# bogus2000/anytime-3D-reconstruction

Measured on AMD Instinct MI355X. Metric: 32^3 voxel reconstructions/sec at batch=256; IoU delta vs reference, higher is better.
Workload: dtype bf16

## Files before the change

### anytime-3d-reconstruction_amd/csrc/conv_direct.hip

```cpp
#include "direct_common.h"

namespace {

constexpr int CD_CIN = 64, CD_COUT = 128;
constexpr int CD_RB = CD_CIN * 2;
constexpr int CD_PIECES = 51;
constexpr int CD_TILE = CD_PIECES * 1024;
constexpr int CD_WST = CD_COUT * 128;
constexpr int CD_NST = 3;
constexpr int CD_RING = 2 * CD_TILE;
constexpr int CD_DUMMY = CD_RING + CD_NST * CD_WST;
constexpr int CD_LDS = CD_DUMMY + 1024;
constexpr int CD_SP = CD_COUT * 2 + 16;

__global__ __launch_bounds__(512, 1) void conv_direct_kernel(const __bf16 *__restrict__ x, const __bf16 *__restrict__ w,
                                                             const float *__restrict__ scale, const float *__restrict__ shift,
                                                             void *__restrict__ y, int dout_log2, unsigned x_bytes, unsigned w_bytes,
                                                             int act, int out_fp8) {
    extern __shared__ __attribute__((aligned(16))) char smem[];
    const int tid = threadIdx.x, lane = tid & 63;
    const int wave = __builtin_amdgcn_readfirstlane(tid >> 6);
    const int wm = wave >> 1, wn = wave & 1;
    const int lo = dout_log2, no = 1 << lo, li = lo + 1, n = 1 << li;

// ... 126 lines not shown
#pragma unroll
        for (int nt = 0; nt < 2; ++nt)
#pragma unroll
            for (int g = 0; g < 4; ++g) shv[nt][g] = *reinterpret_cast<const f32x4 *>(shift + wn * 64 + nt * 32 + 8 * g + 4 * fh);
    }
    auto fill = VV_DIRECT_FILL32(CD_SP, wn * 64);
    auto with_out = [&](auto act_c) {
        if (out_fp8) fill(act_c, std::true_type{});
        else fill(act_c, std::false_type{});
    };
    VV_WITH_ACT(act, with_out);
    __syncthreads();
    vv_direct_store_box<512, CD_SP, CD_COUT, CD_COUT>(stage, y, box, lo, tid, out_fp8);
}

__global__ __launch_bounds__(512, 1) void conv_direct16_kernel(const __bf16 *__restrict__ x, const __bf16 *__restrict__ w,
                                                             const float *__restrict__ scale, const float *__restrict__ shift,
                                                             void *__restrict__ y, int dout_log2, unsigned x_bytes, unsigned w_bytes,
                                                             int act, int out_fp8) {
    extern __shared__ __attribute__((aligned(16))) char smem[];
    const int tid = threadIdx.x, lane = tid & 63;
    const int wave = __builtin_amdgcn_readfirstlane(tid >> 6);
    const int wm = wave >> 1, wn = wave & 1;
    const int lo = dout_log2, no = 1 << lo, li = lo + 1, n = 1 << li;

    const VvDirectBox box = vv_direct_box(no);
    const int b = box.b, od0 = box.od0, oh0 = box.oh0, ow0 = box.ow0;

    const u32x4 rsx = vv_make_rsrc(x, x_bytes), rsw = vv_make_rsrc(w, w_bytes);
    const unsigned lds0 = (unsigned)(unsigned long long)(lptr_t)smem;
// ... 20 lines not shown
            const int g = (lane & 7) ^ ((row >> 1) & 7);
            const unsigned vo = c < 64 ? (unsigned)row * (64 * CD_RB) + t * CD_RB + g * 16 : 0xFFFFFFF0u;
            vv_dma16(rsw, vo, st + (wave * 2 + i) * 1024);
        }
    };

#pragma unroll 1
    for (int s = 0; s < 7; ++s) issue_x(0, s);
    issue_w(0);
    issue_w(1);
    issue_w(2);
    vv_wait_vm<0>();
    __syncthreads();

    const int r = lane & 15, kq = lane >> 4;
    const int rl0 = wm * 81 + (r >> 3) * 9 + (r & 7);
    unsigned xo[2][2], wo[2];
#pragma unroll
    for (int aw = 0; aw < 2; ++aw)
#pragma unroll
        for (int ks = 0; ks < 2; ++ks) xo[aw][ks] = lds0 + rl0 * CD_RB + (((ks * 4 + kq) ^ ((2 * ((r & 7) + aw)) & 7)) << 4);
#pragma unroll
    for (int ks = 0; ks < 2; ++ks) wo[ks] = lds0 + CD_RING + (wn * 64 + r) * 128 + (((ks * 4 + kq) ^ ((r >> 1) & 7)) << 4);

    f32x4 acc[4][4];
#pragma unroll
    for (int i = 0; i < 4; ++i)
#pragma unroll
        for (int j = 0; j < 4; ++j) acc[i][j] = f32x4{0.f, 0.f, 0.f, 0.f};

#define CD16_LD(F, XA, XOFF, WA)                                                                                                    \
// ... 3 lines not shown
                 : "=&v"(F[0]), "=&v"(F[1]), "=&v"(F[2]), "=&v"(F[3]), "=&v"(F[4]), "=&v"(F[5]), "=&v"(F[6]), "=&v"(F[7])            \
                 : "v"(XA), "v"(WA), "n"(XOFF), "n"((XOFF) + 2304), "n"((XOFF) + 4608), "n"((XOFF) + 6912)                          \
                 : "memory")
#define CD16_WAIT(F, N)                                                                                                             \
    asm volatile("s_waitcnt lgkmcnt(%8)"                                                                                            \
                 : "+v"(F[0]), "+v"(F[1]), "+v"(F[2]), "+v"(F[3]), "+v"(F[4]), "+v"(F[5]), "+v"(F[6]), "+v"(F[7])                    \
                 : "n"(N)                                                                                                           \
                 : "memory")
#define CD16_SB __builtin_amdgcn_sched_barrier(0)
#define CD16_RD(D, A, OFF) asm volatile("ds_read_b128 %0, %1 offset:%2" : "=&v"(D) : "v"(A), "n"(OFF) : "memory")
#define CD16_MF(F, COT, CT)                                                                                                         \
    acc[COT][CT] = __builtin_amdgcn_mfma_f32_16x16x32_bf16(*reinterpret_cast<const bf16x8 *>(&F[4 + COT]),                          \
                                                           *reinterpret_cast<const bf16x8 *>(&F[CT]), acc[COT][CT], 0, 0, 0)

    u32x4 P[8], Q[8];
    CD16_LD(P, xo[0][0], 0, wo[0]);

#pragma unroll 1
    for (int q = 0; q < 8; ++q) {
        const unsigned tsel = (q & 1) * CD_TILE, tnext = ((q + 1) & 1) * CD_TILE;
        auto tap = [&](auto a_c) {
            constexpr int A = decltype(a_c)::value;
            constexpr int AW = A & 1, TO = (((A >> 2) & 1) * 81 + ((A >> 1) & 1) * 9 + AW) * CD_RB;
            constexpr int AN = (A + 1) & 7, AWN = AN & 1, TON = (((AN >> 2) & 1) * 81 + ((AN >> 1) & 1) * 9 + AWN) * CD_RB;
            const int c = q * 8 + A;
            const unsigned wsel = (c % CD_NST) * CD_WST, wnext = ((c + 1) % CD_NST) * CD_WST;
            const unsigned xq = xo[AW][1] + tsel, wq = wo[1] + wsel;
            CD16_WAIT(P, 0);
            CD16_SB;
            CD16_MF(P, 0, 0); CD16_MF(P, 0, 1); CD16_SB; CD16_RD(Q[0], xq, TO); CD16_RD(Q[4], wq, 0); CD16_SB;
            CD16_MF(P, 0, 2); CD16_MF(P, 0, 3); CD16_SB; CD16_RD(Q[1], xq, TO + 2304); CD16_RD(Q[5], wq, 2048); CD16_SB;
            CD16_MF(P, 1, 0); CD16_MF(P, 1, 1); CD16_SB; CD16_RD(Q[2], xq, TO + 4608); CD16_RD(Q[6], wq, 4096); CD16_SB;
            CD16_MF(P, 1, 2); CD16_MF(P, 1, 3); CD16_SB; CD16_RD(Q[3], xq, TO + 6912); CD16_RD(Q[7], wq, 6144); CD16_SB;
            CD16_MF(P, 2, 0); CD16_MF(P, 2, 1); CD16_MF(P, 2, 2); CD16_MF(P, 2, 3);
            CD16_MF(P, 3, 0); CD16_MF(P, 3, 1); CD16_MF(P, 3, 2); CD16_MF(P, 3, 3);
            CD16_SB;
            CD16_WAIT(Q, 0);
            vv_wait_vm<(A == 0 || A == 7) ? 2 : 3>();
            __syncthreads();
            CD16_SB;
            CD16_MF(Q, 0, 0); CD16_MF(Q, 0, 1);
// ... 22 lines not shown
    vv_wait_vm<0>();
    __syncthreads();

    char *stage = smem;
    f32x4 scv[4], shv[4];
#pragma unroll
    for (int cot = 0; cot < 4; ++cot) { scv[cot] = f32x4{1.f, 1.f, 1.f, 1.f}; shv[cot] = f32x4{0.f, 0.f, 0.f, 0.f}; }
    if (scale) {
#pragma unroll
        for (int cot = 0; cot < 4; ++cot) scv[cot] = *reinterpret_cast<const f32x4 *>(scale + wn * 64 + cot * 16 + 4 * kq);
    }
    if (shift) {
#pragma unroll
        for (int cot = 0; cot < 4; ++cot) shv[cot] = *reinterpret_cast<const f32x4 *>(shift + wn * 64 + cot * 16 + 4 * kq);
    }
    auto fill = VV_DIRECT_FILL16(CD_SP, wn * 64);
    auto with_out = [&](auto act_c) {
        if (out_fp8) fill(act_c, std::true_type{});
        else fill(act_c, std::false_type{});
    };
    VV_WITH_ACT(act, with_out);
    __syncthreads();
    vv_direct_store_box<512, CD_SP, CD_COUT, CD_COUT>(stage, y, box, lo, tid, out_fp8);
}


constexpr int CDH_COUT = 64;
constexpr int CDH_WST = CDH_COUT * 128;
constexpr int CDH_RING = CD_TILE;
constexpr int CDH_DUMMY = CDH_RING + CD_NST * CDH_WST;
constexpr int CDH_LDS = CDH_DUMMY + 1024;
// ... 136 lines not shown
    vv_wait_vm<0>();
    __syncthreads();

    char *stage = smem;
    f32x4 scv[4], shv[4];
#pragma unroll
    for (int cot = 0; cot < 4; ++cot) { scv[cot] = f32x4{1.f, 1.f, 1.f, 1.f}; shv[cot] = f32x4{0.f, 0.f, 0.f, 0.f}; }
    if (scale) {
#pragma unroll
        for (int cot = 0; cot < 4; ++cot) scv[cot] = *reinterpret_cast<const f32x4 *>(scale + nh * CDH_COUT + cot * 16 + 4 * kq);
    }
    if (shift) {
#pragma unroll
        for (int cot = 0; cot < 4; ++cot) shv[cot] = *reinterpret_cast<const f32x4 *>(shift + nh * CDH_COUT + cot * 16 + 4 * kq);
    }
    auto fill = VV_DIRECT_FILL16(CDH_SP, 0);
    auto with_out = [&](auto act_c) {
        if (out_fp8) fill(act_c, std::true_type{});
        else fill(act_c, std::false_type{});
    };
    VV_WITH_ACT(act, with_out);
    __syncthreads();
    vv_direct_store_box<256, CDH_SP, CDH_COUT, CD_COUT>(stage, y, box, lo, tid, out_fp8);
}


}

VV_EXPORT int vv_conv3d_k4s2_direct_supported(int side, int cin, int cout, int dtype) {
    return dtype == VV_BF16 && cin == CD_CIN && cout == CD_COUT && side >= 16 && vv_is_pow2(side);
}

VV_EXPORT int vv_conv3d_k4s2_direct_fwd_io(const void *x, const void *w_packed, const float *scale, const float *shift, void *y,
                                           int batch, int side, int cin, int cout, int act, int dtype, int out_dtype, void *stream) {
    if (!x || !w_packed || !y) return VV_ERR_NULL;
    if (out_dtype != VV_BF16 && out_dtype != VV_FP8) return VV_ERR_DTYPE;
    if (!vv_conv3d_k4s2_direct_supported(side, cin, cout, dtype) || batch <= 0) return VV_ERR_SHAPE;
    if (!vv_aligned16(x) || !vv_aligned16(w_packed) || !vv_aligned16(y)) return VV_ERR_ALIGN;
    const int so = side / 2;
    const int boxes = (so / 4) * (so / 8) * (so / 8);
    vv_allow_lds<&conv_direct_kernel>(CD_LDS);
    vv_allow_lds<&conv_direct16_kernel>(CD_LDS);
    vv_allow_lds<&conv_direct16h_kernel>(CDH_LDS);
    const int shape = vv_hook_int(vv_hook("VV_CD_SHAPE"), 16);
    const bool s16 = shape != 32, half = shape == 8;
    const size_t in_per = (size_t)side * side * side * cin * 2, out_per = (size_t)so * so * so * cout * (out_dtype == VV_FP8 ? 1 : 2);
    const int per = vv_chunk_samples(in_per, batch);
    if (per < 1) return VV_ERR_SHAPE;
    for (int b0 = 0; b0 < batch; b0 += per) {
        const int nb = batch - b0 < per ? batch - b0 : per;
        const __bf16 *xc = reinterpret_cast<const __bf16 *>(reinterpret_cast<const char *>(x) + (size_t)b0 * in_per);
        void *yc = reinterpret_cast<char *>(y) + (size_t)b0 * out_per;
        if (half)
            VV_LAUNCH(conv_direct16h_kernel, dim3(nb * boxes * 2), dim3(256), CDH_LDS, reinterpret_cast<hipStream_t>(stream), xc,
                      reinterpret_cast<const __bf16 *>(w_packed), scale, shift, yc, vv_log2(so), (unsigned)((size_t)nb * in_per),
                      (unsigned)((size_t)64 * cin * cout * 2), act, out_dtype == VV_FP8 ? 1 : 0,
                      vv_hook_int(vv_hook("VV_CDH_STAGGER"), 5), vv_hook_int(vv_hook("VV_CDH_ABL"), 0));
        else if (s16)
            VV_LAUNCH(conv_direct16_kernel, dim3(nb * boxes), dim3(512), CD_LDS, reinterpret_cast<hipStream_t>(stream), xc,
                      reinterpret_cast<const __bf16 *>(w_packed), scale, shift, yc, vv_log2(so), (unsigned)((size_t)nb * in_per),
                      (unsigned)((size_t)64 * cin * cout * 2), act, out_dtype == VV_FP8 ? 1 : 0);
        else
            VV_LAUNCH(conv_direct_kernel, dim3(nb * boxes), dim3(512), CD_LDS, reinterpret_cast<hipStream_t>(stream), xc,
                      reinterpret_cast<const __bf16 *>(w_packed), scale, shift, yc, vv_log2(so), (unsigned)((size_t)nb * in_per),
                      (unsigned)((size_t)64 * cin * cout * 2), act, out_dtype == VV_FP8 ? 1 : 0);
        const int rc = vv_launch_status();
        if (rc != VV_OK) return rc;
    }
    return VV_OK;
}

VV_EXPORT int vv_conv3d_k4s2_direct_fwd(const void *x, const void *w_packed, const float *scale, const float *shift, void *y,
                                        int batch, int side, int cin, int cout, int act, int dtype, void *stream) {
    return vv_conv3d_k4s2_direct_fwd_io(x, w_packed, scale, shift, y, batch, side, cin, cout, act, dtype, dtype, stream);
// ... 2 lines not shown
```

### anytime-3d-reconstruction_amd/csrc/convt_whole.hip

```cpp

#include <utility>

#include "common.h"

namespace {

constexpr int CW_X = 512 * 256;
constexpr int CW_WST = 64 * 128;
constexpr int CW_NST = 3;
constexpr int CW_RING = CW_X;
constexpr int CW_ZERO = CW_RING + CW_NST * CW_WST;
constexpr int CW_SS = CW_ZERO + 256;
constexpr int CW_LDS = CW_SS + 512;

#define CW_LD(F, X0, X1, WA)                                                                                                     \
    asm volatile("ds_read_b128 %0, %4\n\tds_read_b128 %1, %5\n\tds_read_b128 %2, %6\n\tds_read_b128 %3, %6 offset:4096"          \
                 : "=&v"(F[0]), "=&v"(F[1]), "=&v"(F[2]), "=&v"(F[3])                                                            \
                 : "v"(X0), "v"(X1), "v"(WA)                                                                                     \
                 : "memory")
#define CW_WAIT(F, N) asm volatile("s_waitcnt lgkmcnt(%4)" : "+v"(F[0]), "+v"(F[1]), "+v"(F[2]), "+v"(F[3]) : "n"(N) : "memory")
#define CW_MFMA4(F)                                                                                                              \
    do {                                                                                                                         \
        _Pragma("unroll") for (int nt = 0; nt < 2; ++nt) _Pragma("unroll") for (int mt = 0; mt < 2; ++mt)                        \
            acc[nt][mt] = __builtin_amdgcn_mfma_f32_32x32x16_bf16(*reinterpret_cast<const bf16x8 *>(&F[2 + nt]),                 \
// ... 182 lines not shown
                 "ds_read_b128 %7, %12 offset:6144"                                                                                 \
                 : "=&v"(F[0]), "=&v"(F[1]), "=&v"(F[2]), "=&v"(F[3]), "=&v"(F[4]), "=&v"(F[5]), "=&v"(F[6]), "=&v"(F[7])            \
                 : "v"(XA[0]), "v"(XA[1]), "v"(XA[2]), "v"(XA[3]), "v"(WA)                                                           \
                 : "memory")
#define CW16_WAIT(F, N)                                                                                                             \
    asm volatile("s_waitcnt lgkmcnt(%8)"                                                                                            \
                 : "+v"(F[0]), "+v"(F[1]), "+v"(F[2]), "+v"(F[3]), "+v"(F[4]), "+v"(F[5]), "+v"(F[6]), "+v"(F[7])                    \
                 : "n"(N)                                                                                                           \
                 : "memory")
#define CW16_SB __builtin_amdgcn_sched_barrier(0)
#define CW16_RD(D, A, OFF) asm volatile("ds_read_b128 %0, %1 offset:%2" : "=&v"(D) : "v"(A), "n"(OFF) : "memory")
#define CW16_MF(F, COT, CT)                                                                                                         \
    acc[COT][CT] = __builtin_amdgcn_mfma_f32_16x16x32_bf16(*reinterpret_cast<const bf16x8 *>(&F[4 + COT]),                          \
                                                           *reinterpret_cast<const bf16x8 *>(&F[CT]), acc[COT][CT], 0, 0, 0)

template <int ACT, bool STATS = false>
__global__ __launch_bounds__(512, 1) void ctw16_kernel(const __bf16 *__restrict__ x, const __bf16 *__restrict__ w,
                                                       const float *__restrict__ scale, const float *__restrict__ shift,
                                                       __bf16 *__restrict__ y, int npar, float *__restrict__ partial = nullptr) {
    extern __shared__ __attribute__((aligned(256))) char smem[];
    const int tid = threadIdx.x, lane = tid & 63;
    const int wave = __builtin_amdgcn_readfirstlane(tid >> 6);
    const int ps = 8 / npar;
    const int b = (int)blockIdx.x / ps, p0 = ((int)blockIdx.x % ps) * npar;
    const int NC = npar * 16;
    const unsigned lds0 = (unsigned)(unsigned long long)(lptr_t)smem;

    const u32x4 rsx = vv_make_rsrc(x + (size_t)b * (512 * 128), CW_X);
    const u32x4 rsw = vv_make_rsrc(w, 64 * 128 * 64 * 2);
    {
        const int pos = lane & 15, vsub = lane >> 4;
// ... 13 lines not shown
    issue_w(0, 0);
    issue_w(1, 1);
    issue_w(2, 2);
    if (tid < 16) *reinterpret_cast<uint4 *>(smem + CW_ZERO + tid * 16) = uint4{0u, 0u, 0u, 0u};
    if (tid >= 64 && tid < 128) {
        const int ch = tid - 64;
        *reinterpret_cast<float *>(smem + CW_SS + ch * 4) = scale ? scale[ch] : 1.f;
        *reinterpret_cast<float *>(smem + CW_SS + 256 + ch * 4) = shift ? shift[ch] : 0.f;
    }
    vv_wait_vm<0>();
    __syncthreads();

    const int r = lane & 15, q = lane >> 4;
    const int rh = r >> 3, rw = r & 7;
    const unsigned wl = lds0 + CW_RING + r * 128 + ((q ^ ((r >> 1) & 7)) << 4);
    const unsigned R0 = lds0 + (unsigned)((wave * 64 + r) << 8);
    const unsigned ZR = lds0 + CW_ZERO;
    auto tap_setup = [&](auto a_c, int pd, int ph, int pw, unsigned (&t)[4]) {
        constexpr int A = decltype(a_c)::value;
        const int dd = pd - ((A >> 2) & 1), dh = ph - ((A >> 1) & 1), dw = pw - (A & 1);
        const bool okw = (unsigned)(wave + dd) < 8u && (unsigned)(rw + dw) < 8u;
        const int sft = dd * 64 + dh * 8 + dw;
        const unsigned key = ((unsigned)((2 * (rw + dw)) ^ q) & 15u) << 4;
#pragma unroll
        for (int ct = 0; ct < 4; ++ct) {
            const unsigned row = okw && (unsigned)(2 * ct + rh + dh) < 8u ? R0 + (unsigned)((sft + 16 * ct) << 8) : ZR;
            t[ct] = row ^ key;
        }
    };

    f32x4 acc[4][4];
#pragma unroll
    for (int i = 0; i < 4; ++i)
#pragma unroll
        for (int j = 0; j < 4; ++j) acc[i][j] = f32x4{0.f, 0.f, 0.f, 0.f};
    f32x4 st1[4], st2[4];
#pragma unroll
    for (int i = 0; i < 4; ++i) { st1[i] = f32x4{0.f, 0.f, 0.f, 0.f}; st2[i] = f32x4{0.f, 0.f, 0.f, 0.f}; }

    auto epilogue = [&](int p) {
        const int pd = (p >> 2) & 1, ph = (p >> 1) & 1, pw = p & 1;
        const int qo = (q & 1) * 32 + (q >> 1) * 16;
        char *yb = reinterpret_cast<char *>(y) + ((((size_t)b * 16 + 2 * wave + pd) * 16 + 2 * rh + ph) * 16 + 2 * rw + pw) * 128 + qo;
        const char *ss = smem + CW_SS + q * 16;
#pragma unroll
        for (int c2 = 0; c2 < 2; ++c2) {
            u32x2 o[2][4];
#pragma unroll
            for (int h = 0; h < 2; ++h) {
                const int cot = 2 * c2 + h;
                const f32x4 sc = *reinterpret_cast<const f32x4 *>(ss + cot * 64);
                const f32x4 sh = *reinterpret_cast<const f32x4 *>(ss + 256 + cot * 64);
#pragma unroll
                for (int ct = 0; ct < 4; ++ct) {
                    const f32x4 t = vv_bn_act4<ACT>(acc[cot][ct], sc, sh);
                    bf16x4 v;
#pragma unroll
                    for (int e = 0; e < 4; ++e) v[e] = static_cast<__bf16>(t[e]);
                    if (STATS) {
                        const f32x4 f = {(float)v[0], (float)v[1], (float)v[2], (float)v[3]};
                        st1[cot] += f;
                        st2[cot] += f * f;
                    }
                    acc[cot][ct] = f32x4{0.f, 0.f, 0.f, 0.f};
                    o[h][ct] = *reinterpret_cast<const u32x2 *>(&v);
                }
            }
#pragma unroll
            for (int ct = 0; ct < 4; ++ct) {
                auto rx = __builtin_amdgcn_permlane16_swap(o[0][ct][0], o[1][ct][0], false, false);
                auto ry = __builtin_amdgcn_permlane16_swap(o[0][ct][1], o[1][ct][1], false, false);
                *reinterpret_cast<u32x4 *>(yb + (size_t)(ct * 4 * 16 * 128) + c2 * 64) = u32x4{rx[0], ry[0], rx[1], ry[1]};
            }
        }
    };

    u32x4 P[8], Q[8];
    unsigned ua[4], ub[4];
    tap_setup(std::integral_constant<int, 0>{}, (p0 >> 2) & 1, (p0 >> 1) & 1, p0 & 1, ua);
    unsigned ws = wl;
    int stg = 0, cw = 3;
    CW16_LD(P, ua, ws);
#pragma unroll 1
    for (int pi = 0; pi < npar; ++pi) {
        const int p = p0 + pi, pd = (p >> 2) & 1, ph = (p >> 1) & 1, pw = p & 1;
        const int pn = p + 1, pnd = (pn >> 2) & 1, pnh = (pn >> 1) & 1, pnw = pn & 1;
        auto chunk = [&](auto j_c) {
            constexpr int J = decltype(j_c)::value, A = J >> 1, KH = J & 1;
            unsigned xq[4];
#pragma unroll
            for (int ct = 0; ct < 4; ++ct) xq[ct] = ua[ct] ^ (KH ? 192u : 64u);
            const unsigned wq = ws ^ 64u;
            CW16_WAIT(P, 0);
            CW16_SB;
            CW16_MF(P, 0, 0); CW16_MF(P, 0, 1); CW16_SB; CW16_RD(Q[0], xq[0], 0); CW16_RD(Q[4], wq, 0); CW16_SB;
            CW16_MF(P, 0, 2); CW16_MF(P, 0, 3); CW16_SB; CW16_RD(Q[1], xq[1], 0); CW16_RD(Q[5], wq, 2048); CW16_SB;
            CW16_MF(P, 1, 0); CW16_MF(P, 1, 1); CW16_SB; CW16_RD(Q[2], xq[2], 0); CW16_RD(Q[6], wq, 4096); CW16_SB;
            CW16_MF(P, 1, 2); CW16_MF(P, 1, 3); CW16_SB; CW16_RD(Q[3], xq[3], 0); CW16_RD(Q[7], wq, 6144); CW16_SB;
            CW16_MF(P, 2, 0); CW16_MF(P, 2, 1); CW16_MF(P, 2, 2); CW16_MF(P, 2, 3);
            if (KH == 0) {
                if (A < 7) tap_setup(std::integral_constant<int, (A + 1) & 7>{}, pd, ph, pw, ub);
                else tap_setup(std::integral_constant<int, 0>{}, pnd, pnh, pnw, ub);
// ... 13 lines not shown
            if (KH == 0) {
#pragma unroll
                for (int ct = 0; ct < 4; ++ct) xq[ct] = ua[ct] ^ 128u;
            } else {
#pragma unroll
                for (int ct = 0; ct < 4; ++ct) xq[ct] = ua[ct] = ub[ct];
            }
            CW16_SB;
            CW16_MF(Q, 0, 2); CW16_MF(Q, 0, 3); CW16_SB; CW16_RD(P[0], xq[0], 0); CW16_RD(P[4], ws, 0); CW16_SB;
            CW16_MF(Q, 1, 0); CW16_MF(Q, 1, 1); CW16_SB; CW16_RD(P[1], xq[1], 0); CW16_RD(P[5], ws, 2048); CW16_SB;
            CW16_MF(Q, 1, 2); CW16_MF(Q, 1, 3); CW16_SB; CW16_RD(P[2], xq[2], 0); CW16_RD(P[6], ws, 4096); CW16_SB;
            CW16_MF(Q, 2, 0); CW16_MF(Q, 2, 1); CW16_SB; CW16_RD(P[3], xq[3], 0); CW16_RD(P[7], ws, 6144); CW16_SB;
            CW16_MF(Q, 2, 2); CW16_MF(Q, 2, 3);
            CW16_MF(Q, 3, 0); CW16_MF(Q, 3, 1); CW16_MF(Q, 3, 2); CW16_MF(Q, 3, 3);
            CW16_SB;
        };
        chunk(std::integral_constant<int, 0>{});
        chunk(std::integral_constant<int, 1>{});
        chunk(std::integral_constant<int, 2>{});
        chunk(std::integral_constant<int, 3>{});
        chunk(std::integral_constant<int, 4>{});
        chunk(std::integral_constant<int, 5>{});
        chunk(std::integral_constant<int, 6>{});
        chunk(std::integral_constant<int, 7>{});
        chunk(std::integral_constant<int, 8>{});
        chunk(std::integral_constant<int, 9>{});
        chunk(std::integral_constant<int, 10>{});
        chunk(std::integral_constant<int, 11>{});
        chunk(std::integral_constant<int, 12>{});
        chunk(std::integral_constant<int, 13>{});
// ... 332 lines not shown
    if (!vv_convT3d_k4s2_whole_supported(side, cin, cout, dtype) || batch <= 0) return VV_ERR_SHAPE;
    if (!vv_aligned16(x) || !vv_aligned16(w_skip) || !vv_aligned16(y)) return VV_ERR_ALIGN;
    int ps = 1;
    while (ps < 8 && (long)batch * ps < 256) ps *= 2;
    if (const char *e = vv_hook("VV_CTW_PS")) {
        const int v = atoi(e);
        if (v == 1 || v == 2 || v == 4 || v == 8) ps = v;
    }
    const int shape = vv_hook_int(vv_hook("VV_CTW_SHAPE"), 16);
    const bool shape16 = shape != 32;
    hipStream_t st = reinterpret_cast<hipStream_t>(stream);
    auto launch = [&](auto act_c) {
        constexpr int ACT = decltype(act_c)::value;
        vv_allow_lds<&ctw_kernel<ACT>>(CW_LDS);
        vv_allow_lds<&ctw16_kernel<ACT>>(CW_LDS);
        vv_allow_lds<&ctw4_kernel<ACT>>(CW_LDS);
        if (shape != 16 && shape != 32)
            VV_LAUNCH(ctw4_kernel<ACT>, dim3((unsigned)batch * ps), dim3(256), CW_LDS, st, reinterpret_cast<const __bf16 *>(x),
                      reinterpret_cast<const __bf16 *>(w_skip), scale, shift, reinterpret_cast<__bf16 *>(y), 8 / ps);
        else if (shape16)
            VV_LAUNCH(ctw16_kernel<ACT>, dim3((unsigned)batch * ps), dim3(512), CW_LDS, st, reinterpret_cast<const __bf16 *>(x),
                      reinterpret_cast<const __bf16 *>(w_skip), scale, shift, reinterpret_cast<__bf16 *>(y), 8 / ps);
        else
            VV_LAUNCH(ctw_kernel<ACT>, dim3((unsigned)batch * ps), dim3(512), CW_LDS, st, reinterpret_cast<const __bf16 *>(x),
                      reinterpret_cast<const __bf16 *>(w_skip), scale, shift, reinterpret_cast<__bf16 *>(y), 8 / ps);
    };
    vv_with_act(act, launch);
    return vv_launch_status();
}

VV_EXPORT int vv_convT3d_k4s2_whole_stats_blocks(int batch) { return batch > 0 ? batch : 0; }

VV_EXPORT int vv_convT3d_k4s2_whole_stats_fwd(const void *x, const void *w_skip, void *y, float *stats_partial, size_t stats_bytes, int batch,
// ... 12 lines not shown
```

### anytime-3d-reconstruction_amd/csrc/direct_common.h

```cpp
#pragma once
#include "common.h"

struct VvDirectBox { int b, od0, oh0, ow0, nh; };

template <bool HALVES = false>
__device__ __forceinline__ VvDirectBox vv_direct_box(int no) {
    const int nwg = gridDim.x;
    int blk = (nwg & 7) == 0 ? (int)(blockIdx.x & 7) * (nwg >> 3) + (int)(blockIdx.x >> 3) : (int)blockIdx.x;
    VvDirectBox o;
    o.nh = 0;
    if (HALVES) { o.nh = blk & 1; blk >>= 1; }
    const int bxw = no >> 3, bxh = no >> 3, bxd = no >> 2;
    const int bw = blk % bxw; blk /= bxw;
    const int bh = blk % bxh; blk /= bxh;
    const int bd = blk % bxd;
    o.b = blk / bxd;
    o.od0 = bd * 4; o.oh0 = bh * 8; o.ow0 = bw * 8;
    return o;
}

#define VV_DIRECT_PUT4(dst, c, v)                                                                          \
    do {                                                                                                   \
        if (FP8) {                                                                                         \
            *reinterpret_cast<unsigned *>(dst + c) = vv_pack_fp8x4(v);                                     \
        } else {                                                                                           \
            bf16x4 o;                                                                                      \
            _Pragma("unroll") for (int e = 0; e < 4; ++e) o[e] = static_cast<__bf16>(v[e]);                \
            *reinterpret_cast<bf16x4 *>(dst + c * 2) = o;                                                  \
        }                                                                                                  \
    } while (0)

#define VV_DIRECT_FILL16(PITCH, C0)                                                                        \
    [&](auto act_c, auto fp8_c) {                                                                          \
        constexpr int ACT = decltype(act_c)::value;                                                        \
        constexpr bool FP8 = decltype(fp8_c)::value;                                                       \
        _Pragma("unroll") for (int ct = 0; ct < 4; ++ct)                                                   \
            _Pragma("unroll") for (int cot = 0; cot < 4; ++cot) {                                          \
                const int c = (C0) + cot * 16 + 4 * kq;                                                    \
                const f32x4 sc = scv[cot], sh = shv[cot];                                                  \
                const f32x4 v = vv_bn_act4<ACT>(acc[cot][ct], sc, sh);                                     \
                char *dst = stage + (wm * 64 + ct * 16 + r) * (PITCH);                                     \
                VV_DIRECT_PUT4(dst, c, v);                                                                 \
            }                                                                                              \
    }
#define VV_DIRECT_FILL32(PITCH, C0)                                                                        \
    [&](auto act_c, auto fp8_c) {                                                                          \
        constexpr int ACT = decltype(act_c)::value;                                                        \
        constexpr bool FP8 = decltype(fp8_c)::value;                                                       \
        _Pragma("unroll") for (int mt = 0; mt < 2; ++mt)                                                   \
            _Pragma("unroll") for (int nt = 0; nt < 2; ++nt)                                               \
                _Pragma("unroll") for (int g = 0; g < 4; ++g) {                                            \
                    const int c = (C0) + nt * 32 + 8 * g + 4 * fh;                                         \
                    const f32x4 sc = scv[nt][g], sh = shv[nt][g];                                          \
                    f32x4 v;                                                                               \
                    _Pragma("unroll") for (int e = 0; e < 4; ++e) {                                        \
                        float t = acc[nt][mt][4 * g + e] * sc[e] + sh[e];                                  \
// ... 23 lines not shown
```

### anytime-3d-reconstruction_amd/csrc/skip_direct.hip

```cpp
#include "common.h"

namespace {

typedef __attribute__((ext_vector_type(4))) unsigned sd_u4;

constexpr int SD_ATILE = 256 * 128;
constexpr int SD_WST = 32768;
constexpr int SD_A0 = 4096;
constexpr int SD_W0 = SD_A0 + 2 * SD_ATILE;
constexpr int SD_ZERO = SD_W0 + 2 * SD_WST;
constexpr int SD_LDS = SD_ZERO + 4096;
constexpr int SD_XCH = 0;
constexpr int SD_OST = 65536;
constexpr int SD_OPITCH = 144;
constexpr int SD_TPITCH = 272;
constexpr int SD_TWAVE = 16 * SD_TPITCH;

struct SdArgs {
    const void *x;
    const void *w;
    const float *scale;
    const float *shift;
    void *y;
    int batch, cin, cout, act;
// ... 86 lines not shown
}

__global__ void sd_pack_convT_multi_kernel(const SdPackJobs t) {
    int j = 0;
    while (j + 1 < t.njobs && (int)blockIdx.x >= t.first[j + 1]) ++j;
    sd_pack_convT_body(t.w[j], t.out[j], t.cin[j], t.cout[j], (int)blockIdx.x - t.first[j], t.first[j + 1] - t.first[j]);
}

#define SD_RD(DST, ADDR, OFF) asm volatile("ds_read_b128 %0, %1 offset:%2" : "=v"(DST) : "v"(ADDR), "n"(OFF) : "memory")
#define SD_WAIT8(N, F, G)                                                                                                   \
    asm volatile("s_waitcnt lgkmcnt(%8)"                                                                                    \
                 : "+v"(F[0]), "+v"(F[1]), "+v"(F[2]), "+v"(F[3]), "+v"(G[0]), "+v"(G[1]), "+v"(G[2]), "+v"(G[3])          \
                 : "n"(N)                                                                                                   \
                 : "memory")

template <int MODE>
__global__ __launch_bounds__(512, 1) void sd_kernel(const SdArgs a) {
    extern __shared__ __attribute__((aligned(16))) char smem[];
    const int tid = threadIdx.x, lane = tid & 63;
    const int wave = __builtin_amdgcn_readfirstlane(tid >> 6);
    const int mq = wave & 3, hv = wave >> 2;
    const int NC = a.cin >> 6;

    const int nwg = gridDim.x;
    const int wi = (nwg & 7) ? (int)blockIdx.x : (int)(blockIdx.x & 7) * (nwg >> 3) + (int)(blockIdx.x >> 3);
    const int sg = wi / a.groups, g = wi - sg * a.groups;
    const int b0 = sg * 4;
    const int ng = MODE == 0 ? g : (g >> 2);
    const int pd = (g >> 1) & 1, ph = g & 1;

    const u32x4 rsx = vv_make_rsrc(a.x, a.x_bytes), rsw = vv_make_rsrc(a.w, a.w_bytes);
    const unsigned lds0 = (unsigned)(unsigned long long)(lptr_t)smem;

    for (int i = tid; i < 256; i += 512) reinterpret_cast<uint4 *>(smem + SD_ZERO)[i] = make_uint4(0, 0, 0, 0);
    __syncthreads();

// ... 274 lines not shown
    __builtin_amdgcn_s_barrier();

    const int kq4 = kq * 4;
    if constexpr (MODE == 0) {
        f32x4 *xch = reinterpret_cast<f32x4 *>(smem + SD_XCH);
        {
            f32x4 *mine = xch + (size_t)wave * 8 * 64 + lane;
#pragma unroll
            for (int i = 0; i < 4; ++i)
#pragma unroll
                for (int j = 0; j < 2; ++j) mine[(i * 2 + j) * 64] = hv ? acc[i][j] : acc[i][2 + j];
        }
        __syncthreads();
        f32x4 fin[4][2];
        {
            const f32x4 *theirs = xch + (size_t)(wave ^ 4) * 8 * 64 + lane;
#pragma unroll
            for (int i = 0; i < 4; ++i)
#pragma unroll
                for (int j = 0; j < 2; ++j) fin[i][j] = (hv ? acc[i][2 + j] : acc[i][j]) + theirs[(i * 2 + j) * 64];
        }
        f32x4 sc[2], sh[2];
#pragma unroll
        for (int j = 0; j < 2; ++j) {
            const int n = ng * 64 + (2 * hv + j) * 16 + kq4;
            sc[j] = a.scale ? *reinterpret_cast<const f32x4 *>(a.scale + n) : f32x4{1.f, 1.f, 1.f, 1.f};
            sh[j] = a.shift ? *reinterpret_cast<const f32x4 *>(a.shift + n) : f32x4{0.f, 0.f, 0.f, 0.f};
        }
        auto fill = [&](auto act_c) {
            constexpr int ACT = decltype(act_c)::value;
#pragma unroll
// ... 60 lines not shown
                    if (b < a.batch)
                        *reinterpret_cast<uint4 *>(reinterpret_cast<char *>(a.y) + ((((size_t)b * 8 + od) * 8 + oh) * 8 + ow) * (a.cout * 2) + ng * 256 + pc * 16) =
                            *reinterpret_cast<const uint4 *>(mystage + row * SD_TPITCH + pc * 16);
                }
                asm volatile("s_waitcnt lgkmcnt(0)" ::: "memory");
                __builtin_amdgcn_wave_barrier();
            }
        };
        VV_WITH_ACT(a.act, fill);
    }
}

template <int MODE>
int sd_launch(const void *x, const void *w, const float *scale, const float *shift, void *y, int batch, int cin, int cout, int act,
              hipStream_t st) {
    vv_allow_lds<&sd_kernel<MODE>>(SD_LDS);
    const size_t in_vox = MODE == 0 ? 512 : 64, out_vox = MODE == 0 ? 64 : 512;
    const size_t sample_in = in_vox * cin * 2, sample_out = out_vox * cout * 2;
    int per = (int)((0x7FFFFFFFull / sample_in) & ~3ull);
    if (per < 4) return VV_ERR_SHAPE;
    for (int s0 = 0; s0 < batch; s0 += per) {
        const int nb = batch - s0 < per ? batch - s0 : per;
        SdArgs a;
        a.x = reinterpret_cast<const char *>(x) + (size_t)s0 * sample_in;
        a.y = reinterpret_cast<char *>(y) + (size_t)s0 * sample_out;
        a.w = w; a.scale = scale; a.shift = shift;
        a.batch = nb; a.cin = cin; a.cout = cout; a.act = act;
        a.x_bytes = (unsigned)((size_t)nb * sample_in);
        a.w_bytes = (unsigned)((size_t)64 * cin * cout * 2);
        a.groups = MODE == 0 ? cout / 64 : 4 * (cout / 128);
        const int nsg = (nb + 3) / 4;
        VV_LAUNCH(sd_kernel<MODE>, dim3(nsg * a.groups), dim3(512), SD_LDS, st, a);
        const int rc = vv_launch_status();
        if (rc != VV_OK) return rc;
    }
    return VV_OK;
}

}

VV_EXPORT int vv_conv3d_k4s2_skip_supported(int side, int cin, int cout, int dtype) {
    return dtype == VV_BF16 && side == 8 && cin >= 64 && cin % 64 == 0 && cout >= 64 && cout % 64 == 0 && (size_t)64 * cin * cout * 2 < 0xFFFFFFF0ull;
}

VV_EXPORT int vv_convT3d_k4s2_skip_supported(int side, int cin, int cout, int dtype) {
    return dtype == VV_BF16 && side == 4 && cin >= 64 && cin % 64 == 0 && cout >= 128 && cout % 128 == 0 && (size_t)64 * cin * cout * 2 < 0xFFFFFFF0ull;
}
// ... 78 lines not shown
```

### anytime-3d-reconstruction_amd/voxvae/lib.py

```python
import ctypes
import os

import torch

PKG = os.path.dirname(os.path.dirname(os.path.abspath(__file__)))
LIB_PATH = os.path.join(PKG, 'lib', 'libvoxvae.so')
HOOKS_LIB_PATH = os.path.join(PKG, 'lib', 'libvoxvae_hooks.so')
HOOK_VARS = ('VV_CD_SHAPE', 'VV_CDH_STAGGER', 'VV_CDH_ABL', 'VV_DIRECT_MT', 'VV_LT_KSLICE', 'VV_SPLIT_TARGET', 'VV_SPLIT_MINCHUNKS', 'VV_NO_KHALVES', 'VV_POSMAJOR_CONV_SIDE',
             'VV_POSMAJOR_CONVT_SIDE', 'VV_STAGES', 'VV_NO_FIRSTCONV', 'VV_WGRAD_F32', 'VV_PG_TARGET', 'VV_CTW_PS', 'VV_CTW_SHAPE',
             'VV_NO_WGRAD_PHASE', 'VV_BN_NB', 'VV_BN_SWEEP', 'VV_FINAL_BCE', 'VV_FIRSTCONV_GATHER', 'VV_FIRSTCONV_WGS', 'VV_FIRSTCONV_NOCHAIN', 'VV_CHUNK_SAMPLES')

VV_F32, VV_BF16, VV_FP8 = 0, 1, 2
ACT = {None: 0, 'None': 0, 'linear': 0, 'elu': 1, 'relu': 2, 'lrelu': 3}
DTYPES = {'f32': VV_F32, 'fp32': VV_F32, 'float32': VV_F32, 'bf16': VV_BF16, 'bfloat16': VV_BF16, 'fp8': VV_FP8}

_vp, _i, _f, _sz, _l = ctypes.c_void_p, ctypes.c_int, ctypes.c_float, ctypes.c_size_t, ctypes.c_long

SIGNATURES = {
    'vv_abi_version': (_i, []),
    'vv_status_string': (ctypes.c_char_p, [_i]),
    'vv_last_hip_error': (ctypes.c_char_p, []),
    'vv_pack_conv_k4': (_i, [_vp, _vp, _i, _i, _i, _vp]),
    'vv_pack_convT_k4s2': (_i, [_vp, _vp, _i, _i, _i, _vp]),
    'vv_pack_conv_k4s1_meanpool': (_i, [_vp, _vp, _i, _i, _i, _i, _vp]),
    'vv_pack_conv_k4s1_full': (_i, [_vp, _vp, _i, _i, _i, _i, _vp]),
# ... 151 lines not shown
```

Before: 560,700.

## Deal output tiles diagonally across waves to skip out-of-range boundary taps

The default 16-wide direct conv kernel now maps each wave's four column tiles onto rotated depth planes, so boundary planes are spread across waves. Whole MFMA groups for depth taps that fall outside the volume can then be skipped per wave instead of being multiplied against padding. The epilogue row mapping and LDS read addresses are rewritten to match. An opt-in diagonal variant of the transposed-conv kernel (shape hook 1) and a hook-gated wave remap for the skip kernel are also added; these add code paths and risk new LDS bank conflicts or branch overhead.

```diff
diff --git a/anytime-3d-reconstruction_amd/csrc/conv_direct.hip b/anytime-3d-reconstruction_amd/csrc/conv_direct.hip
--- a/anytime-3d-reconstruction_amd/csrc/conv_direct.hip
+++ b/anytime-3d-reconstruction_amd/csrc/conv_direct.hip
@@ -164,6 +164,7 @@
     vv_direct_store_box<512, CD_SP, CD_COUT, CD_COUT>(stage, y, box, lo, tid, out_fp8);
 }
 
+template <bool DEAL>
 __global__ __launch_bounds__(512, 1) void conv_direct16_kernel(const __bf16 *__restrict__ x, const __bf16 *__restrict__ w,
                                                              const float *__restrict__ scale, const float *__restrict__ shift,
                                                              void *__restrict__ y, int dout_log2, unsigned x_bytes, unsigned w_bytes,
@@ -214,7 +215,11 @@
     __syncthreads();
 
     const int r = lane & 15, kq = lane >> 4;
-    const int rl0 = wm * 81 + (r >> 3) * 9 + (r & 7);
+    const int rl0 = (DEAL ? 0 : wm * 81) + (r >> 3) * 9 + (r & 7);
+    int shp[4];
+    unsigned shb[4];
+#pragma unroll
+    for (int ct = 0; ct < 4; ++ct) { shp[ct] = DEAL ? (ct + wm) & 3 : ct; shb[ct] = (unsigned)(shp[ct] * 2304); }
     unsigned xo[2][2], wo[2];
 #pragma unroll
     for (int aw = 0; aw < 2; ++aw)
@@ -248,7 +253,14 @@
                                                            *reinterpret_cast<const bf16x8 *>(&F[CT]), acc[COT][CT], 0, 0, 0)
 
     u32x4 P[8], Q[8];
-    CD16_LD(P, xo[0][0], 0, wo[0]);
+    const bool skip_lo = DEAL && od0 == 0, skip_hi = DEAL && od0 + 4 == no;
+    if constexpr (DEAL) {
+        CD16_RD(P[0], xo[0][0] + shb[0], 0); CD16_RD(P[1], xo[0][0] + shb[1], 81 * CD_RB); CD16_RD(P[2], xo[0][0] + shb[2], 2 * 81 * CD_RB);
+        CD16_RD(P[3], xo[0][0] + shb[3], 3 * 81 * CD_RB);
+        CD16_RD(P[4], wo[0], 0); CD16_RD(P[5], wo[0], 2048); CD16_RD(P[6], wo[0], 4096); CD16_RD(P[7], wo[0], 6144);
+    } else {
+        CD16_LD(P, xo[0][0], 0, wo[0]);
+    }
 
 #pragma unroll 1
     for (int q = 0; q < 8; ++q) {
@@ -259,6 +271,41 @@
             constexpr int AN = (A + 1) & 7, AWN = AN & 1, TON = (((AN >> 2) & 1) * 81 + ((AN >> 1) & 1) * 9 + AWN) * CD_RB;
             const int c = q * 8 + A;
             const unsigned wsel = (c % CD_NST) * CD_WST, wnext = ((c + 1) % CD_NST) * CD_WST;
+            if constexpr (DEAL) {
+                constexpr int AD = (A >> 2) & 1, CS = AD ? 3 : 0, N0 = CS == 0 ? 1 : 0, N1 = N0 + 1, N2 = N0 + 2;
+                constexpr int PL = 81 * CD_RB;
+                const bool sk = AD ? skip_hi && (q & 4) : skip_lo && !(q & 4);
+                const unsigned xb = xo[AW][1] + tsel, wq = wo[1] + wsel;
+                const unsigned xq0 = xb + shb[0], xq1 = xb + shb[1], xq2 = xb + shb[2], xq3 = xb + shb[3];
+                CD16_WAIT(P, 0);
+                CD16_SB;
+                CD16_MF(P, 0, N0); CD16_MF(P, 0, N1); CD16_SB; CD16_RD(Q[0], xq0, TO); CD16_RD(Q[4], wq, 0); CD16_SB;
+                CD16_MF(P, 0, N2); CD16_MF(P, 1, N0); CD16_SB; CD16_RD(Q[1], xq1, TO + PL); CD16_RD(Q[5], wq, 2048); CD16_SB;
+                CD16_MF(P, 1, N1); CD16_MF(P, 1, N2); CD16_SB; CD16_RD(Q[2], xq2, TO + 2 * PL); CD16_RD(Q[6], wq, 4096); CD16_SB;
+                CD16_MF(P, 2, N0); CD16_MF(P, 2, N1); CD16_SB; CD16_RD(Q[3], xq3, TO + 3 * PL); CD16_RD(Q[7], wq, 6144); CD16_SB;
+                CD16_MF(P, 2, N2); CD16_MF(P, 3, N0); CD16_MF(P, 3, N1); CD16_MF(P, 3, N2);
+                CD16_SB;
+                if (!sk) { CD16_MF(P, 0, CS); CD16_MF(P, 1, CS); CD16_MF(P, 2, CS); CD16_MF(P, 3, CS); CD16_SB; }
+                CD16_WAIT(Q, 0);
+                vv_wait_vm<(A == 0 || A == 7) ? 2 : 3>();
+                __syncthreads();
+                CD16_SB;
+                CD16_MF(Q, 0, N0); CD16_MF(Q, 0, N1);
+                if (A < 7) issue_x(q + 1, A);
+                CD16_MF(Q, 0, N2); CD16_MF(Q, 1, N0);
+                issue_w(c + 3);
+                const unsigned xn = xo[AWN][0] + (A == 7 ? tnext : tsel), wp = wo[0] + wnext;
+                const unsigned xp0 = xn + shb[0], xp1 = xn + shb[1], xp2 = xn + shb[2], xp3 = xn + shb[3];
+                CD16_SB;
+                CD16_RD(P[0], xp0, TON); CD16_RD(P[4], wp, 0); CD16_SB;
+                CD16_MF(Q, 1, N1); CD16_MF(Q, 1, N2); CD16_SB; CD16_RD(P[1], xp1, TON + PL); CD16_RD(P[5], wp, 2048); CD16_SB;
+                CD16_MF(Q, 2, N0); CD16_MF(Q, 2, N1); CD16_SB; CD16_RD(P[2], xp2, TON + 2 * PL); CD16_RD(P[6], wp, 4096); CD16_SB;
+                CD16_MF(Q, 2, N2); CD16_MF(Q, 3, N0); CD16_SB; CD16_RD(P[3], xp3, TON + 3 * PL); CD16_RD(P[7], wp, 6144); CD16_SB;
+                CD16_MF(Q, 3, N1); CD16_MF(Q, 3, N2);
+                CD16_SB;
+                if (!sk) { CD16_MF(Q, 0, CS); CD16_MF(Q, 1, CS); CD16_MF(Q, 2, CS); CD16_MF(Q, 3, CS); CD16_SB; }
+                return;
+            }
             const unsigned xq = xo[AW][1] + tsel, wq = wo[1] + wsel;
             CD16_WAIT(P, 0);
             CD16_SB;
@@ -311,7 +358,7 @@
 #pragma unroll
         for (int cot = 0; cot < 4; ++cot) shv[cot] = *reinterpret_cast<const f32x4 *>(shift + wn * 64 + cot * 16 + 4 * kq);
     }
-    auto fill = VV_DIRECT_FILL16(CD_SP, wn * 64);
+    auto fill = VV_DIRECT_FILL16(CD_SP, wn * 64, (DEAL ? ct * 64 + shp[ct] * 16 : wm * 64 + ct * 16) + r);
     auto with_out = [&](auto act_c) {
         if (out_fp8) fill(act_c, std::true_type{});
         else fill(act_c, std::false_type{});
@@ -478,7 +525,7 @@
 #pragma unroll
         for (int cot = 0; cot < 4; ++cot) shv[cot] = *reinterpret_cast<const f32x4 *>(shift + nh * CDH_COUT + cot * 16 + 4 * kq);
     }
-    auto fill = VV_DIRECT_FILL16(CDH_SP, 0);
+    auto fill = VV_DIRECT_FILL16(CDH_SP, 0, wm * 64 + ct * 16 + r);
     auto with_out = [&](auto act_c) {
         if (out_fp8) fill(act_c, std::true_type{});
         else fill(act_c, std::false_type{});
@@ -504,7 +551,8 @@
     const int so = side / 2;
     const int boxes = (so / 4) * (so / 8) * (so / 8);
     vv_allow_lds<&conv_direct_kernel>(CD_LDS);
-    vv_allow_lds<&conv_direct16_kernel>(CD_LDS);
+    vv_allow_lds<&conv_direct16_kernel<true>>(CD_LDS);
+    vv_allow_lds<&conv_direct16_kernel<false>>(CD_LDS);
     vv_allow_lds<&conv_direct16h_kernel>(CDH_LDS);
     const int shape = vv_hook_int(vv_hook("VV_CD_SHAPE"), 16);
     const bool s16 = shape != 32, half = shape == 8;
@@ -520,8 +568,12 @@
                       reinterpret_cast<const __bf16 *>(w_packed), scale, shift, yc, vv_log2(so), (unsigned)((size_t)nb * in_per),
                       (unsigned)((size_t)64 * cin * cout * 2), act, out_dtype == VV_FP8 ? 1 : 0,
                       vv_hook_int(vv_hook("VV_CDH_STAGGER"), 5), vv_hook_int(vv_hook("VV_CDH_ABL"), 0));
+        else if (shape == 1)
+            VV_LAUNCH(conv_direct16_kernel<false>, dim3(nb * boxes), dim3(512), CD_LDS, reinterpret_cast<hipStream_t>(stream), xc,
+                      reinterpret_cast<const __bf16 *>(w_packed), scale, shift, yc, vv_log2(so), (unsigned)((size_t)nb * in_per),
+                      (unsigned)((size_t)64 * cin * cout * 2), act, out_dtype == VV_FP8 ? 1 : 0);
         else if (s16)
-            VV_LAUNCH(conv_direct16_kernel, dim3(nb * boxes), dim3(512), CD_LDS, reinterpret_cast<hipStream_t>(stream), xc,
+            VV_LAUNCH(conv_direct16_kernel<true>, dim3(nb * boxes), dim3(512), CD_LDS, reinterpret_cast<hipStream_t>(stream), xc,
                       reinterpret_cast<const __bf16 *>(w_packed), scale, shift, yc, vv_log2(so), (unsigned)((size_t)nb * in_per),
                       (unsigned)((size_t)64 * cin * cout * 2), act, out_dtype == VV_FP8 ? 1 : 0);
         else
diff --git a/anytime-3d-reconstruction_amd/csrc/convt_whole.hip b/anytime-3d-reconstruction_amd/csrc/convt_whole.hip
--- a/anytime-3d-reconstruction_amd/csrc/convt_whole.hip
+++ b/anytime-3d-reconstruction_amd/csrc/convt_whole.hip
@@ -220,7 +220,7 @@
     acc[COT][CT] = __builtin_amdgcn_mfma_f32_16x16x32_bf16(*reinterpret_cast<const bf16x8 *>(&F[4 + COT]),                          \
                                                            *reinterpret_cast<const bf16x8 *>(&F[CT]), acc[COT][CT], 0, 0, 0)
 
-template <int ACT, bool STATS = false>
+template <int ACT, bool STATS = false, bool DEAL = false>
 __global__ __launch_bounds__(512, 1) void ctw16_kernel(const __bf16 *__restrict__ x, const __bf16 *__restrict__ w,
                                                        const float *__restrict__ scale, const float *__restrict__ shift,
                                                        __bf16 *__restrict__ y, int npar, float *__restrict__ partial = nullptr) {
@@ -264,18 +264,36 @@
     const int r = lane & 15, q = lane >> 4;
     const int rh = r >> 3, rw = r & 7;
     const unsigned wl = lds0 + CW_RING + r * 128 + ((q ^ ((r >> 1) & 7)) << 4);
-    const unsigned R0 = lds0 + (unsigned)((wave * 64 + r) << 8);
+    static_assert(!(STATS && DEAL), "the statistics form keeps the wave-per-plane mapping");
+    int sd[4], shp[4];
+#pragma unroll
+    for (int ct = 0; ct < 4; ++ct) {
+        shp[ct] = DEAL ? (wave + ((0x1320 >> (4 * ct)) & 3)) & 3 : ct;
+        sd[ct] = DEAL ? (wave - shp[ct]) & 7 : wave;
+    }
+    const bool has0 = DEAL && sd[0] == 0, has7 = DEAL && sd[3] == 7;
+    const unsigned R0 = DEAL ? lds0 + (unsigned)(r << 8) : lds0 + (unsigned)((wave * 64 + r) << 8);
     const unsigned ZR = lds0 + CW_ZERO;
     auto tap_setup = [&](auto a_c, int pd, int ph, int pw, unsigned (&t)[4]) {
         constexpr int A = decltype(a_c)::value;
         const int dd = pd - ((A >> 2) & 1), dh = ph - ((A >> 1) & 1), dw = pw - (A & 1);
-        const bool okw = (unsigned)(wave + dd) < 8u && (unsigned)(rw + dw) < 8u;
         const int sft = dd * 64 + dh * 8 + dw;
         const unsigned key = ((unsigned)((2 * (rw + dw)) ^ q) & 15u) << 4;
-#pragma unroll
-        for (int ct = 0; ct < 4; ++ct) {
-            const unsigned row = okw && (unsigned)(2 * ct + rh + dh) < 8u ? R0 + (unsigned)((sft + 16 * ct) << 8) : ZR;
-            t[ct] = row ^ key;
+        if constexpr (DEAL) {
+            const bool okw = (unsigned)(rw + dw) < 8u;
+#pragma unroll
+            for (int ct = 0; ct < 4; ++ct) {
+                const bool ok = okw && (unsigned)(sd[ct] + dd) < 8u && (unsigned)(2 * shp[ct] + rh + dh) < 8u;
+                const unsigned row = ok ? R0 + (unsigned)((sft + 64 * sd[ct] + 16 * shp[ct]) << 8) : ZR;
+                t[ct] = row ^ key;
+            }
+        } else {
+            const bool okw = (unsigned)(wave + dd) < 8u && (unsigned)(rw + dw) < 8u;
+#pragma unroll
+            for (int ct = 0; ct < 4; ++ct) {
+                const unsigned row = okw && (unsigned)(2 * ct + rh + dh) < 8u ? R0 + (unsigned)((sft + 16 * ct) << 8) : ZR;
+                t[ct] = row ^ key;
+            }
         }
     };
 
@@ -292,6 +310,11 @@
         const int pd = (p >> 2) & 1, ph = (p >> 1) & 1, pw = p & 1;
         const int qo = (q & 1) * 32 + (q >> 1) * 16;
         char *yb = reinterpret_cast<char *>(y) + ((((size_t)b * 16 + 2 * wave + pd) * 16 + 2 * rh + ph) * 16 + 2 * rw + pw) * 128 + qo;
+        char *ybs[4];
+#pragma unroll
+        for (int ct = 0; ct < 4; ++ct)
+            ybs[ct] = reinterpret_cast<char *>(y) + ((((size_t)b * 16 + 2 * sd[ct] + pd) * 16 + 4 * shp[ct] + ph) * 16 + pw) * 128;
+        const unsigned yl = (unsigned)(((2 * rh) * 16 + 2 * rw) * 128 + qo);
         const char *ss = smem + CW_SS + q * 16;
 #pragma unroll
         for (int c2 = 0; c2 < 2; ++c2) {
@@ -320,7 +343,8 @@
             for (int ct = 0; ct < 4; ++ct) {
                 auto rx = __builtin_amdgcn_permlane16_swap(o[0][ct][0], o[1][ct][0], false, false);
                 auto ry = __builtin_amdgcn_permlane16_swap(o[0][ct][1], o[1][ct][1], false, false);
-                *reinterpret_cast<u32x4 *>(yb + (size_t)(ct * 4 * 16 * 128) + c2 * 64) = u32x4{rx[0], ry[0], rx[1], ry[1]};
+                char *dst = DEAL ? ybs[ct] + (yl + c2 * 64) : yb + (size_t)(ct * 4 * 16 * 128) + c2 * 64;
+                *reinterpret_cast<u32x4 *>(dst) = u32x4{rx[0], ry[0], rx[1], ry[1]};
             }
         }
     };
@@ -335,7 +359,57 @@
     for (int pi = 0; pi < npar; ++pi) {
         const int p = p0 + pi, pd = (p >> 2) & 1, ph = (p >> 1) & 1, pw = p & 1;
         const int pn = p + 1, pnd = (pn >> 2) & 1, pnh = (pn >> 1) & 1, pnw = pn & 1;
-        auto chunk = [&](auto j_c) {
+        const bool skip_lo = has7 && pd == 1, skip_hi = has0 && pd == 0;
+        auto chunk_deal = [&](auto j_c) {
+            constexpr int J = decltype(j_c)::value, A = J >> 1, KH = J & 1, CS = ((A >> 2) & 1) ? 0 : 3;
+            constexpr int N0 = CS == 0 ? 1 : 0, N1 = N0 + 1, N2 = N0 + 2;
+            const bool sk = ((A >> 2) & 1) ? skip_hi : skip_lo;
+            unsigned xq[4];
+#pragma unroll
+            for (int ct = 0; ct < 4; ++ct) xq[ct] = ua[ct] ^ (KH ? 192u : 64u);
+            const unsigned wq = ws ^ 64u;
+            CW16_WAIT(P, 0);
+            CW16_SB;
+            CW16_MF(P, 0, N0); CW16_MF(P, 0, N1); CW16_SB; CW16_RD(Q[0], xq[0], 0); CW16_RD(Q[4], wq, 0); CW16_SB;
+            CW16_MF(P, 0, N2); CW16_MF(P, 1, N0); CW16_SB; CW16_RD(Q[1], xq[1], 0); CW16_RD(Q[5], wq, 2048); CW16_SB;
+            CW16_MF(P, 1, N1); CW16_MF(P, 1, N2); CW16_SB; CW16_RD(Q[2], xq[2], 0); CW16_RD(Q[6], wq, 4096); CW16_SB;
+            CW16_MF(P, 2, N0); CW16_MF(P, 2, N1); CW16_SB; CW16_RD(Q[3], xq[3], 0); CW16_RD(Q[7], wq, 6144); CW16_SB;
+            CW16_MF(P, 2, N2); CW16_MF(P, 3, N0);
+            if (KH == 0) {
+                if (A < 7) tap_setup(std::integral_constant<int, (A + 1) & 7>{}, pd, ph, pw, ub);
+                else tap_setup(std::integral_constant<int, 0>{}, pnd, pnh, pnw, ub);
+                asm volatile("" : "+v"(ub[0]), "+v"(ub[1]), "+v"(ub[2]), "+v"(ub[3]));
+            }
+            CW16_MF(P, 3, N1); CW16_MF(P, 3, N2);
+            CW16_SB;
+            if (!sk) { CW16_MF(P, 0, CS); CW16_MF(P, 1, CS); CW16_MF(P, 2, CS); CW16_MF(P, 3, CS); CW16_SB; }
+            CW16_WAIT(Q, 0);
+            if (J < 2 && pi > 0) vv_wait_vm<9>();
+            else vv_wait_vm<1>();
+            __builtin_amdgcn_s_barrier();
+            CW16_SB;
+            CW16_MF(Q, 0, N0); CW16_MF(Q, 0, N1); CW16_SB;
+            issue_w(cw, stg);
+            ++cw;
+            stg = stg == CW_NST - 1 ? 0 : stg + 1;
+            ws = wl + stg * CW_WST;
+            if (KH == 0) {
+#pragma unroll
+                for (int ct = 0; ct < 4; ++ct) xq[ct] = ua[ct] ^ 128u;
+            } else {
+#pragma unroll
+                for (int ct = 0; ct < 4; ++ct) xq[ct] = ua[ct] = ub[ct];
+            }
+            CW16_SB;
+            CW16_MF(Q, 0, N2); CW16_MF(Q, 1, N0); CW16_SB; CW16_RD(P[0], xq[0], 0); CW16_RD(P[4], ws, 0); CW16_SB;
+            CW16_MF(Q, 1, N1); CW16_MF(Q, 1, N2); CW16_SB; CW16_RD(P[1], xq[1], 0); CW16_RD(P[5], ws, 2048); CW16_SB;
+            CW16_MF(Q, 2, N0); CW16_MF(Q, 2, N1); CW16_SB; CW16_RD(P[2], xq[2], 0); CW16_RD(P[6], ws, 4096); CW16_SB;
+            CW16_MF(Q, 2, N2); CW16_MF(Q, 3, N0); CW16_SB; CW16_RD(P[3], xq[3], 0); CW16_RD(P[7], ws, 6144); CW16_SB;
+            CW16_MF(Q, 3, N1); CW16_MF(Q, 3, N2);
+            CW16_SB;
+            if (!sk) { CW16_MF(Q, 0, CS); CW16_MF(Q, 1, CS); CW16_MF(Q, 2, CS); CW16_MF(Q, 3, CS); CW16_SB; }
+        };
+        auto chunk_plane = [&](auto j_c) {
             constexpr int J = decltype(j_c)::value, A = J >> 1, KH = J & 1;
             unsigned xq[4];
 #pragma unroll
@@ -379,6 +453,10 @@
             CW16_MF(Q, 2, 2); CW16_MF(Q, 2, 3);
             CW16_MF(Q, 3, 0); CW16_MF(Q, 3, 1); CW16_MF(Q, 3, 2); CW16_MF(Q, 3, 3);
             CW16_SB;
+        };
+        auto chunk = [&](auto j_c) {
+            if constexpr (DEAL) chunk_deal(j_c);
+            else chunk_plane(j_c);
         };
         chunk(std::integral_constant<int, 0>{});
         chunk(std::integral_constant<int, 1>{});
@@ -741,9 +819,13 @@
         constexpr int ACT = decltype(act_c)::value;
         vv_allow_lds<&ctw_kernel<ACT>>(CW_LDS);
         vv_allow_lds<&ctw16_kernel<ACT>>(CW_LDS);
+        vv_allow_lds<&ctw16_kernel<ACT, false, true>>(CW_LDS);
         vv_allow_lds<&ctw4_kernel<ACT>>(CW_LDS);
-        if (shape != 16 && shape != 32)
+        if (shape != 16 && shape != 32 && shape != 1)
             VV_LAUNCH(ctw4_kernel<ACT>, dim3((unsigned)batch * ps), dim3(256), CW_LDS, st, reinterpret_cast<const __bf16 *>(x),
+                      reinterpret_cast<const __bf16 *>(w_skip), scale, shift, reinterpret_cast<__bf16 *>(y), 8 / ps);
+        else if (shape == 1)
+            VV_LAUNCH((ctw16_kernel<ACT, false, true>), dim3((unsigned)batch * ps), dim3(512), CW_LDS, st, reinterpret_cast<const __bf16 *>(x),
                       reinterpret_cast<const __bf16 *>(w_skip), scale, shift, reinterpret_cast<__bf16 *>(y), 8 / ps);
         else if (shape16)
             VV_LAUNCH(ctw16_kernel<ACT>, dim3((unsigned)batch * ps), dim3(512), CW_LDS, st, reinterpret_cast<const __bf16 *>(x),
diff --git a/anytime-3d-reconstruction_amd/csrc/direct_common.h b/anytime-3d-reconstruction_amd/csrc/direct_common.h
--- a/anytime-3d-reconstruction_amd/csrc/direct_common.h
+++ b/anytime-3d-reconstruction_amd/csrc/direct_common.h
@@ -30,7 +30,7 @@
         }                                                                                                  \
     } while (0)
 
-#define VV_DIRECT_FILL16(PITCH, C0)                                                                        \
+#define VV_DIRECT_FILL16(PITCH, C0, ROW)                                                                     \
     [&](auto act_c, auto fp8_c) {                                                                          \
         constexpr int ACT = decltype(act_c)::value;                                                        \
         constexpr bool FP8 = decltype(fp8_c)::value;                                                       \
@@ -39,7 +39,7 @@
                 const int c = (C0) + cot * 16 + 4 * kq;                                                    \
                 const f32x4 sc = scv[cot], sh = shv[cot];                                                  \
                 const f32x4 v = vv_bn_act4<ACT>(acc[cot][ct], sc, sh);                                     \
-                char *dst = stage + (wm * 64 + ct * 16 + r) * (PITCH);                                     \
+                char *dst = stage + (ROW) * (PITCH);                                                       \
                 VV_DIRECT_PUT4(dst, c, v);                                                                 \
             }                                                                                              \
     }
diff --git a/anytime-3d-reconstruction_amd/csrc/skip_direct.hip b/anytime-3d-reconstruction_amd/csrc/skip_direct.hip
--- a/anytime-3d-reconstruction_amd/csrc/skip_direct.hip
+++ b/anytime-3d-reconstruction_amd/csrc/skip_direct.hip
@@ -124,12 +124,12 @@
                  : "n"(N)                                                                                                   \
                  : "memory")
 
-template <int MODE>
+template <int MODE, bool DIAG2>
 __global__ __launch_bounds__(512, 1) void sd_kernel(const SdArgs a) {
     extern __shared__ __attribute__((aligned(16))) char smem[];
     const int tid = threadIdx.x, lane = tid & 63;
     const int wave = __builtin_amdgcn_readfirstlane(tid >> 6);
-    const int mq = wave & 3, hv = wave >> 2;
+    const int hv = wave >> 2, mq = (wave + (DIAG2 ? 2 * hv : 0)) & 3;
     const int NC = a.cin >> 6;
 
     const int nwg = gridDim.x;
@@ -434,7 +434,7 @@
         __syncthreads();
         f32x4 fin[4][2];
         {
-            const f32x4 *theirs = xch + (size_t)(wave ^ 4) * 8 * 64 + lane;
+            const f32x4 *theirs = xch + (size_t)(wave ^ (DIAG2 ? 6 : 4)) * 8 * 64 + lane;
 #pragma unroll
             for (int i = 0; i < 4; ++i)
 #pragma unroll
@@ -525,7 +525,9 @@
 template <int MODE>
 int sd_launch(const void *x, const void *w, const float *scale, const float *shift, void *y, int batch, int cin, int cout, int act,
               hipStream_t st) {
-    vv_allow_lds<&sd_kernel<MODE>>(SD_LDS);
+    vv_allow_lds<&sd_kernel<MODE, true>>(SD_LDS);
+    vv_allow_lds<&sd_kernel<MODE, false>>(SD_LDS);
+    const bool diag2 = vv_hook_int(vv_hook("VV_SD_DIAG"), 0) != 0;
     const size_t in_vox = MODE == 0 ? 512 : 64, out_vox = MODE == 0 ? 64 : 512;
     const size_t sample_in = in_vox * cin * 2, sample_out = out_vox * cout * 2;
     int per = (int)((0x7FFFFFFFull / sample_in) & ~3ull);
@@ -541,7 +543,8 @@
         a.w_bytes = (unsigned)((size_t)64 * cin * cout * 2);
         a.groups = MODE == 0 ? cout / 64 : 4 * (cout / 128);
         const int nsg = (nb + 3) / 4;
-        VV_LAUNCH(sd_kernel<MODE>, dim3(nsg * a.groups), dim3(512), SD_LDS, st, a);
+        if (diag2) VV_LAUNCH((sd_kernel<MODE, true>), dim3(nsg * a.groups), dim3(512), SD_LDS, st, a);
+        else VV_LAUNCH((sd_kernel<MODE, false>), dim3(nsg * a.groups), dim3(512), SD_LDS, st, a);
         const int rc = vv_launch_status();
         if (rc != VV_OK) return rc;
     }
diff --git a/anytime-3d-reconstruction_amd/voxvae/lib.py b/anytime-3d-reconstruction_amd/voxvae/lib.py
--- a/anytime-3d-reconstruction_amd/voxvae/lib.py
+++ b/anytime-3d-reconstruction_amd/voxvae/lib.py
@@ -8,7 +8,7 @@
 HOOKS_LIB_PATH = os.path.join(PKG, 'lib', 'libvoxvae_hooks.so')
 HOOK_VARS = ('VV_CD_SHAPE', 'VV_CDH_STAGGER', 'VV_CDH_ABL', 'VV_DIRECT_MT', 'VV_LT_KSLICE', 'VV_SPLIT_TARGET', 'VV_SPLIT_MINCHUNKS', 'VV_NO_KHALVES', 'VV_POSMAJOR_CONV_SIDE',
              'VV_POSMAJOR_CONVT_SIDE', 'VV_STAGES', 'VV_NO_FIRSTCONV', 'VV_WGRAD_F32', 'VV_PG_TARGET', 'VV_CTW_PS', 'VV_CTW_SHAPE',
-             'VV_NO_WGRAD_PHASE', 'VV_BN_NB', 'VV_BN_SWEEP', 'VV_FINAL_BCE', 'VV_FIRSTCONV_GATHER', 'VV_FIRSTCONV_WGS', 'VV_FIRSTCONV_NOCHAIN', 'VV_CHUNK_SAMPLES')
+             'VV_NO_WGRAD_PHASE', 'VV_BN_NB', 'VV_BN_SWEEP', 'VV_FINAL_BCE', 'VV_FIRSTCONV_GATHER', 'VV_FIRSTCONV_WGS', 'VV_FIRSTCONV_NOCHAIN', 'VV_CHUNK_SAMPLES', 'VV_SD_DIAG')
 
 VV_F32, VV_BF16, VV_FP8 = 0, 1, 2
 ACT = {None: 0, 'None': 0, 'linear': 0, 'elu': 1, 'relu': 2, 'lrelu': 3}
```

Result: no change. 562,000 (median of 2 runs) (+0.2%).
